# arangesh/TrackMPNN

Measured on AMD Instinct MI355X. Metric: graph_edges_per_sec_fwd_bwd, higher is better.
Workload: dtype f32; 1 GPU; C2 KITTI Car/RRC-shaped rolling windows: 7 frames, D_t~clip(Poisson(6),1,20), F=8 (2d), H=64, K=0, diff; 1 fwd per frame + 1 bwd per window; 16384 windows/GPU batched block-diagonally (64 distinct seeds tiled); windows_per_gpu=16384, rows_final=6762496, parallelism=sequence-dp1

## Files before the change

include/tmpnn.h:

```cpp
#ifndef TMPNN_H
#define TMPNN_H

#include <stddef.h>
#include <stdint.h>

#ifdef __cplusplus
extern "C" {
#endif

#define TMPNN_ABI_VERSION 4

#define TMPNN_OK 0
#define TMPNN_EINVAL (-1)
#define TMPNN_ELAUNCH (-2)
#define TMPNN_EWORKSPACE (-3)

typedef void* tmpnn_stream;
typedef void* tmpnn_event;

typedef struct tmpnn_seg_plan {
    int32_t T;
    int32_t I;
    int32_t nsplit;
    const int32_t* t_row;
// ... 82 lines not shown
int tmpnn_gru_fwd_head_parts(int H, int IN, int xmode);
int tmpnn_gru_fwd(const int32_t* rows, int R, int xmode, const int32_t* src, const int32_t* dst,
                  const float* msg, int ld_msg, int msg_compact, int IN, const float* h, int ld_h, int H,
                  const float* wih_t, const float* whh_t, const float* b_ih, const float* b_hh,
                  float* h_out, int ld_out, float* gates, size_t gate_plane,
                  const float* w_head, float* logit_part, size_t part_stride, tmpnn_stream stream);
int tmpnn_gru_bwd_data(const int32_t* rows, int R, int IN, const float* h, int ld_h, int H,
                       const float* w_ih, const float* w_hh,
                       const float* gates, size_t gate_plane, const float* d_hout, int ld_dhout,
                       const float* dy, const float* w_head,
                       float* d_msg, int ld_dmsg, float* d_h, int ld_dh,
                       const int32_t* add_src, const int32_t* add_dst, const float* add_msg, int ld_add,
                       tmpnn_stream stream);
size_t tmpnn_gru_bwd_weights_ws(int R, int IN, int H);
int tmpnn_gru_bwd_weights(const int32_t* rows, int R, int xmode, const int32_t* src, const int32_t* dst,
                          const float* msg, int ld_msg, int msg_compact, int IN,
                          const float* h, int ld_h, int H,
                          const float* gates, size_t gate_plane, const float* d_hout, int ld_dhout,
                          const float* dy, const float* w_head,
                          float* dW_ih, float* dW_hh, float* db_ih, float* db_hh,
                          void* ws, size_t ws_bytes, tmpnn_stream stream);

int tmpnn_gru_bwd_fused_available(int H, int IN, int xmode);
size_t tmpnn_gru_bwd_fused_ws(int R, int IN, int H);
int tmpnn_gru_bwd_fused(const int32_t* rows, int R, int xmode, const int32_t* src, const int32_t* dst,
                        const float* msg, int ld_msg, int msg_compact, int IN,
                        const float* h, int ld_h, int H, const float* w_ih, const float* w_hh,
                        const float* gates, size_t gate_plane, const float* d_hout, int ld_dhout,
                        const float* dy, const float* w_head,
                        float* d_msg, int ld_dmsg, float* d_h, int ld_dh,
                        const int32_t* add_src, const int32_t* add_dst, const float* add_msg, int ld_add,
                        float* dW_ih, float* dW_hh, float* db_ih, float* db_hh,
                        void* ws, size_t ws_bytes, tmpnn_stream stream);

int tmpnn_gru_fwd_tiles(const tmpnn_edge_tiles* tiles, int R, const float* proj, int ld_proj, const float* h, int ld_h, int H,
                        const float* whh_t, const float* b_ih, const float* b_hh, float* h_out, int ld_out, float* gates,
                        size_t gate_plane, const float* w_head, float* logit_part, size_t part_stride, tmpnn_stream stream);

int tmpnn_rows_linear(const int32_t* rows, int R, const float* in, int ld_in, int H, const float* wt, int NOUT,
                      float* out, int ld_out, tmpnn_stream stream);

int tmpnn_transpose(const float* in, int rows, int cols, float* out, tmpnn_stream stream);

int tmpnn_input_bn_fwd(const float* xdet, int ld_x, int F, int nd, const int32_t* seg_ptr,
                       const int32_t* seg_cnt, const int32_t* seg_of_det ,
                       int S, int H, int training,
                       const float* w1, const float* b1, const float* gamma, const float* beta,
                       float* running_mean, float* running_var,
                       const float* w2, const float* b2,
                       float* y_save, float* mean, float* rstd, float* ws_a ,
                       const int32_t* out_row, float* h_new, int ld_h, tmpnn_stream stream);
size_t tmpnn_input_bn_bwd_ws(int nd, int S, int H, int F);
int tmpnn_input_bn_bwd(const float* xdet, int ld_x, int F, int nd, const int32_t* seg_ptr,
                       const int32_t* seg_cnt, const int32_t* seg_of_det, int S, int H, int training,
                       const float* w1, const float* b1, const float* gamma, const float* beta,
                       const float* w2,
                       const float* y_save, const float* mean, const float* rstd,
                       const int32_t* out_row, const float* d_h, int ld_dh,
                       float* d_xdet, int ld_dx, float* d_xzero,
                       float* dw1, float* db1, float* dgamma, float* dbeta, float* dw2, float* db2,
                       float* ws, size_t ws_floats, tmpnn_stream stream);

int tmpnn_input_tf_supported(int H, int F, int max_seg_rows);
int tmpnn_input_tf_fwd(const float* xdet, const int64_t* x_rows, int ld_x, int F, int nd, const int32_t* seg_ptr, const int32_t* seg_cnt,
                       const int32_t* seg_of_det, int S, int max_seg_rows, int H, int training, const float* w1, const float* b1,
                       const float* gamma, const float* beta, float* running_mean, float* running_var, const float* w2,
// ... 219 lines not shown
```

trackmpnn_amd/_lib.py:

```python
from __future__ import annotations

import ctypes as C

import torch
import os
import re
from typing import Dict, List, Optional

_HERE = os.path.dirname(os.path.abspath(__file__))
LIB_PATH = os.environ.get('TMPNN_LIB_PATH') or os.path.join(_HERE, 'lib', 'libtmpnn.so')
HEADER_PATH = os.path.join(os.path.dirname(_HERE), 'include', 'tmpnn.h')

ABI_VERSION = 4

c_int = C.c_int
c_void_p = C.c_void_p
c_size_t = C.c_size_t
c_float = C.c_float


class CSegPlan(C.Structure):
    _fields_ = [('T', C.c_int32), ('I', C.c_int32), ('nsplit', C.c_int32), ('t_row', c_void_p), ('items', c_void_p),
                ('rowptr2', c_void_p), ('inc2', c_void_p), ('ws', c_void_p), ('ws_floats', c_size_t)]

# ... 60 lines not shown
    'tmpnn_segsum_bwd': (c_int, [_GP, c_void_p, c_int, c_void_p, c_int, c_int, c_int, c_void_p]),
    'tmpnn_att_fwd': (c_int, [_GP, c_void_p, c_void_p, c_int, c_int, c_int, c_void_p, c_void_p, c_void_p, c_float,
                              c_void_p, c_void_p, c_void_p, c_void_p, c_void_p, c_void_p, c_int, c_void_p]),
    'tmpnn_att_bwd_ws': (c_size_t, [c_int, c_int, c_int, c_int]),
    'tmpnn_att_index': (c_int, [_GP, c_void_p, c_void_p, c_void_p, c_void_p, c_void_p, c_void_p]),
    'tmpnn_att_bwd': (c_int, [_GP, c_void_p, c_void_p, c_void_p, c_int, c_int, c_int, c_void_p, c_void_p, c_void_p,
                              c_float, c_void_p, c_void_p, c_void_p, c_void_p, c_void_p, c_int, c_void_p, c_size_t,
                              c_void_p, c_int, c_void_p, c_void_p, c_void_p]),
    'tmpnn_att_bwd_heads': (c_int, [_GP, c_void_p, c_void_p, c_void_p, c_int, c_int, c_int, c_void_p, c_void_p,
                                    c_void_p, c_float, c_void_p, c_void_p, c_void_p, c_void_p, c_void_p, c_int, c_void_p,
                                    c_size_t, c_void_p, c_int, c_void_p, c_void_p, c_void_p]),
    'tmpnn_gru_fwd': (c_int, [c_void_p, c_int, c_int, c_void_p, c_void_p, c_void_p, c_int, c_int, c_int,
                              c_void_p, c_int, c_int, c_void_p, c_void_p, c_void_p, c_void_p,
                              c_void_p, c_int, c_void_p, c_size_t, c_void_p, c_void_p, c_size_t, c_void_p]),
    'tmpnn_gru_fwd_head_parts': (c_int, [c_int, c_int, c_int]),
    'tmpnn_gru_fwd_tiles': (c_int, [_TP, c_int, c_void_p, c_int, c_void_p, c_int, c_int, c_void_p, c_void_p, c_void_p,
                                    c_void_p, c_int, c_void_p, c_size_t, c_void_p, c_void_p, c_size_t, c_void_p]),
    'tmpnn_heads_finish': (c_int, [c_void_p, c_size_t, c_int, c_int, c_void_p, c_void_p, c_void_p, c_void_p, c_void_p, c_void_p]),
    'tmpnn_gru_bwd_data': (c_int, [c_void_p, c_int, c_int, c_void_p, c_int, c_int, c_void_p, c_void_p,
                                   c_void_p, c_size_t, c_void_p, c_int, c_void_p, c_void_p,
                                   c_void_p, c_int, c_void_p, c_int,
                                   c_void_p, c_void_p, c_void_p, c_int, c_void_p]),
    'tmpnn_gru_bwd_weights_ws': (c_size_t, [c_int, c_int, c_int]),
    'tmpnn_gru_bwd_weights': (c_int, [c_void_p, c_int, c_int, c_void_p, c_void_p, c_void_p, c_int, c_int, c_int,
                                      c_void_p, c_int, c_int, c_void_p, c_size_t, c_void_p, c_int, c_void_p, c_void_p,
                                      c_void_p, c_void_p, c_void_p, c_void_p, c_void_p, c_size_t, c_void_p]),
    'tmpnn_gru_bwd_fused_available': (c_int, [c_int, c_int, c_int]),
    'tmpnn_gru_bwd_fused_ws': (c_size_t, [c_int, c_int, c_int]),
    'tmpnn_gru_bwd_fused': (c_int, [c_void_p, c_int, c_int, c_void_p, c_void_p, c_void_p, c_int, c_int, c_int,
                                    c_void_p, c_int, c_int, c_void_p, c_void_p, c_void_p, c_size_t, c_void_p, c_int,
                                    c_void_p, c_void_p, c_void_p, c_int, c_void_p, c_int,
                                    c_void_p, c_void_p, c_void_p, c_int, c_void_p, c_void_p, c_void_p, c_void_p,
                                    c_void_p, c_size_t, c_void_p]),
    'tmpnn_rows_linear': (c_int, [c_void_p, c_int, c_void_p, c_int, c_int, c_void_p, c_int, c_void_p, c_int, c_void_p]),
    'tmpnn_transpose': (c_int, [c_void_p, c_int, c_int, c_void_p, c_void_p]),
    'tmpnn_input_bn_fwd': (c_int, [c_void_p, c_int, c_int, c_int, c_void_p, c_void_p, c_void_p, c_int, c_int, c_int,
                                   c_void_p, c_void_p, c_void_p, c_void_p, c_void_p, c_void_p, c_void_p, c_void_p,
                                   c_void_p, c_void_p, c_void_p, c_void_p, c_void_p, c_void_p, c_int, c_void_p]),
    'tmpnn_input_bn_bwd_ws': (c_size_t, [c_int, c_int, c_int, c_int]),
    'tmpnn_input_bn_bwd': (c_int, [c_void_p, c_int, c_int, c_int, c_void_p, c_void_p, c_void_p, c_int, c_int, c_int,
                                   c_void_p, c_void_p, c_void_p, c_void_p, c_void_p,
                                   c_void_p, c_void_p, c_void_p, c_void_p, c_void_p, c_int,
                                   c_void_p, c_int, c_void_p,
                                   c_void_p, c_void_p, c_void_p, c_void_p, c_void_p, c_void_p,
                                   c_void_p, c_size_t, c_void_p]),
    'tmpnn_input_tf_supported': (c_int, [c_int, c_int, c_int]),
    'tmpnn_input_tf_fwd': (c_int, [c_void_p, c_void_p, c_int, c_int, c_int, c_void_p, c_void_p, c_void_p, c_int, c_int, c_int, c_int,
                                   c_void_p, c_void_p, c_void_p, c_void_p, c_void_p, c_void_p, c_void_p, c_void_p,
                                   c_void_p, c_void_p, c_void_p, c_void_p, c_void_p, c_int, c_void_p]),
    'tmpnn_input_tf_bwd_ws': (c_size_t, [c_int, c_int, c_int, c_int, c_int]),
    'tmpnn_input_tf_bwd': (c_int, [c_void_p, c_void_p, c_int, c_int, c_int, c_void_p, c_void_p, c_void_p, c_int, c_int, c_int, c_int,
                                   c_void_p, c_void_p, c_void_p, c_void_p, c_void_p,
                                   c_void_p, c_void_p, c_void_p, c_void_p, c_void_p, c_int,
                                   c_void_p, c_int, c_void_p,
                                   c_void_p, c_void_p, c_void_p, c_void_p, c_void_p, c_void_p,
                                   c_void_p, c_size_t, c_void_p]),
    'tmpnn_heads_fwd': (c_int, [c_void_p, c_int, c_int, c_int, c_void_p, c_void_p, c_void_p, c_void_p, c_void_p,
                                c_void_p, c_void_p, c_void_p]),
    'tmpnn_heads_bwd_ws': (c_size_t, [c_int, c_int]),
    'tmpnn_heads_bwd': (c_int, [c_void_p, c_int, c_int, c_int, c_void_p, c_void_p, c_void_p, c_void_p, c_void_p,
                                c_void_p, c_void_p, c_void_p, c_int, c_int, c_void_p, c_void_p, c_void_p, c_void_p,
                                c_void_p, c_size_t, c_void_p]),
    'tmpnn_targets': (c_int, [_GP, c_void_p, c_void_p, c_void_p]),
    'tmpnn_ce_loss_ws': (c_size_t, [c_int]),
    'tmpnn_ce_loss_fwd': (c_int, [_GP, c_void_p, c_void_p, c_void_p, c_void_p, c_void_p, c_size_t, c_void_p]),
    'tmpnn_ce_loss_bwd': (c_int, [_GP, c_void_p, c_void_p, c_void_p, c_void_p, c_void_p, c_void_p, c_void_p]),
# ... 149 lines not shown
```

trackmpnn_amd/csrc/gru_bwd.hip:

```cpp
#include "gru_common.h"

namespace tmpnn {



template <int NT>
__global__ __launch_bounds__(256) void k_gru_bwd_data(GruBwdDataArgs a) {
    const int wave = threadIdx.x >> 6, lane = threadIdx.x & 63;
    const int c = lane & 31, half = lane >> 5;
    const int r0 = (blockIdx.x * 4 + wave) * 32;
    if (r0 >= a.R) return;
    const int H = a.H;
    const int vcol0 = blockIdx.y * (32 * NT);
    const bool is_dx = vcol0 < a.IN;
    const int n0 = is_dx ? vcol0 : vcol0 - a.IN;
    const float* __restrict__ W = is_dx ? a.w_ih : a.w_hh;
    const int ldw = is_dx ? a.IN : H;
    const int li = min(r0 + c, a.R - 1);
    const int row = a.rows[li];
    const size_t gp = a.gate_plane;

    f32x16 acc[NT];
#pragma unroll
    for (int t = 0; t < NT; ++t)
// ... 1741 lines not shown
    }
#undef TWO_STAGE
#undef TWO_GATHER_IDS
#undef TWO_ISSUE_GATHER
#undef TWO_ISSUE_MAIN
#undef TWO_SLICE
    float* sw = a.slab_w + (size_t)blockIdx.x * (3 * H) * (2 * H);
    if (HHS || role == 0) {
#pragma unroll
        for (int j = 0; j < 3; ++j)
#pragma unroll
            for (int reg = 0; reg < 16; ++reg) {
                const int jj = (jt0 + j) * 32 + acc_row(reg, half);
                sw[(size_t)jj * (2 * H) + role * H + tt * 32 + c32] = acc[j][reg];
            }
    }
    {
        float* red = lds;
#pragma unroll
        for (int j = 0; j < 3; ++j) {
            const float tot = bsum[j] + __shfl_xor(bsum[j], 32);
            if (half == 0) red[wave * 96 + j * 32 + c32] = tot;
        }
        __syncthreads();
        if (HHS && tt == 0 && half == 0) {
            float* sb = a.slab_b + (size_t)blockIdx.x * 6 * H;
#pragma unroll
            for (int j = 0; j < 3; ++j)
                sb[role * 3 * H + (jt0 + j) * 32 + c32] = red[wave * 96 + j * 32 + c32] + red[(wave + 1) * 96 + j * 32 + c32];
        }
    }
}


__global__ void k_gru_reduce_w(const float* __restrict__ slab_w, const float* __restrict__ slab_b, int n_rs,
                               int IN, int H, float* __restrict__ dW_ih, float* __restrict__ dW_hh,
                               float* __restrict__ db_ih, float* __restrict__ db_hh) {
    const int XH = IN + H;
    const size_t nW = (size_t)3 * H * XH;
    const size_t i = (size_t)blockIdx.x * blockDim.x + threadIdx.x;
    if (i < nW) {
        float s = 0.f;
        for (int k = 0; k < n_rs; ++k) s += slab_w[(size_t)k * nW + i];
        const int j = (int)(i / XH), col = (int)(i % XH);
        if (col < IN) dW_ih[(size_t)j * IN + col] += s;
        else dW_hh[(size_t)j * H + (col - IN)] += s;
    } else if (i < nW + (size_t)6 * H) {
        const int b = (int)(i - nW);
        float s = 0.f;
        for (int k = 0; k < n_rs; ++k) s += slab_b[(size_t)k * 6 * H + b];
        if (b < 3 * H) db_ih[b] += s;
        else db_hh[b - 3 * H] += s;
    }
}

__global__ void k_gru_reduce_w_half(const float* __restrict__ slab_w, const float* __restrict__ slab_b, int n_rs, int H,
                                    float* __restrict__ dW_ih, int ld_dwih, float* __restrict__ dW_hh,
                                    float* __restrict__ db_ih, float* __restrict__ db_hh, int full) {
    const int XH = 2 * H;
    const size_t nW = (size_t)3 * H * XH;
    const size_t i = (size_t)blockIdx.x * blockDim.x + threadIdx.x;
    if (i < nW) {
        const int j = (int)(i / XH), col = (int)(i % XH);
        if (col >= H && !full) return;
        float s = 0.f;
        for (int k = 0; k < n_rs; ++k) s += slab_w[(size_t)k * nW + i];
        if (col < H) dW_ih[(size_t)j * ld_dwih + col] += s;
        else dW_hh[(size_t)j * H + (col - H)] += s;
    } else if (full && i < nW + (size_t)6 * H) {
        const int b = (int)(i - nW);
        float s = 0.f;
        for (int k = 0; k < n_rs; ++k) s += slab_b[(size_t)k * 6 * H + b];
        if (b < 3 * H) db_ih[b] += s;
        else db_hh[b - 3 * H] += s;
    }
}

__global__ void k_fold_slabs_gru(const float* __restrict__ slabs, size_t stride, int nslab, float* __restrict__ out,
                                 size_t n) {
    const size_t i = (size_t)blockIdx.x * blockDim.x + threadIdx.x;
    if (i >= n) return;
    const int k0 = blockIdx.y * 32, k1 = min(nslab, k0 + 32);
    float s = 0.f;
#pragma unroll 8
    for (int k = k0; k < k1; ++k) s += slabs[(size_t)k * stride + i];
    out[(size_t)blockIdx.y * n + i] = s;
}


static int weights_variant_default() {
    static const int v = [] {
        if (!split_enabled()) return 0;
        const char* e = getenv("TMPNN_SPLIT_WEIGHTS");
        return (e && e[0] == '0') ? 0 : 1;
    }();
    return v;
}
static void plan_weights(int R, int IN, int H, int* n_rs, int* RS, int* NQ, int* NCH) {
    *NQ = 3 * H / 32;
    *NCH = (IN + H + 127) / 128;
    long per = (long)(*NQ) * (*NCH);
    long want = 4096 / per;
    if (want < 1) want = 1;
    long by_rows = (R + 63) / 64;
    long n = by_rows < want ? by_rows : want;
    if (n < 1) n = 1;
    long rs = (R + n - 1) / n;
    rs = (rs + 1) & ~1L;
    if (rs < 2) rs = 2;
    n = (R + rs - 1) / rs;
    if (n < 1) n = 1;
    *n_rs = (int)n;
    *RS = (int)rs;
}

}

using namespace tmpnn;

// ... 226 lines not shown
    } while (0)
#else
    TM_REQUIRE(!(xmode == 0 && fuse), "gru_bwd_fused: xmode 0 with a fused adjoint needs a TMPNN_KEEP_VARIANTS build");
#define LF(X, U, F)                                                                                          \
    do {                                                                                                     \
        if (!((X) == 0 && (F))) {                                                                            \
            TM_SHM_ONCE((k_gru_bwd_two<X, U, F>), shm);                                                      \
            hipLaunchKernelGGL((k_gru_bwd_two<X, U, F>), dim3(n_rs), dim3(512), shm, st, a, ntiles);         \
        }                                                                                                    \
    } while (0)
#endif
#define LU(X, F) do { if (up == 1) LF(X, 1, F); else if (up == 2) LF(X, 2, F); else LF(X, 3, F); } while (0)
    if (xmode == 0) { if (fuse) LU(0, true); else LU(0, false); }
    else            { if (fuse) LU(1, true); else LU(1, false); }
#undef LU
#undef LF
    int rc = check_launch("gru_bwd_fused");
    if (rc) return rc;
    const float* rw = slab_w;
    const float* rb = slab_b;
    int nred = n_rs;
    if (n_rs > 64) {
        const int ng = ceil_div(n_rs, 32);
        float* fw = fold;
        float* fb = fold + (size_t)ng * nW;
        hipLaunchKernelGGL(k_fold_slabs_gru, dim3(ceil_div((long)nW, 256), ng), dim3(256), 0, st, slab_w, nW, n_rs, fw, nW);
        hipLaunchKernelGGL(k_fold_slabs_gru, dim3(ceil_div((long)nB, 256), ng), dim3(256), 0, st, slab_b, nB, n_rs, fb, nB);
        if ((rc = check_launch("gru_fold"))) return rc;
        rw = fw; rb = fb; nred = ng;
    }
    hipLaunchKernelGGL(k_gru_reduce_w, dim3(ceil_div((long)(nW + nB), 256)), dim3(256), 0, st, rw, rb, nred, IN, H,
                       dW_ih, dW_hh, db_ih, db_hh);
    return check_launch("gru_reduce_w");
}

#ifdef TMPNN_KEEP_VARIANTS
int tmpnn_gru_bwd_weights_choice(void) { return weights_variant_default(); }
#endif

size_t tmpnn_gru_bwd_weights_ws(int R, int IN, int H) {
    if (R <= 0) return 0;
    int n_rs, RS, NQ, NCH;
    plan_weights(R, IN, H, &n_rs, &RS, &NQ, &NCH);
    if (weights_use_lds(IN, H)) n_rs = std::max(n_rs, weights_lds_blocks(R));
    if (weights_use_chunk(IN, H)) n_rs = std::max(n_rs, weights_chunk_slabs(R, IN, H));
    const size_t per = (size_t)3 * H * (IN + H) + (size_t)6 * H;
    return ((size_t)n_rs * per + reduce_slabs_ws_floats(n_rs, per)) * sizeof(float);
}

int tmpnn_gru_bwd_weights(const int32_t* rows, int R, int xmode, const int32_t* src, const int32_t* dst,
                          const float* msg, int ld_msg, int msg_compact, int IN, const float* h, int ld_h, int H,
                          const float* gates,
                          size_t gate_plane, const float* d_hout, int ld_dhout, const float* dy, const float* w_head,
                          float* dW_ih, float* dW_hh,
                          float* db_ih, float* db_hh, void* ws, size_t ws_bytes, tmpnn_stream stream) {
    return tmpnn_gru_bwd_weights_variant(rows, R, xmode, src, dst, msg, ld_msg, msg_compact, IN, h, ld_h, H, gates,
                                         gate_plane, d_hout, ld_dhout, dy, w_head, dW_ih, dW_hh, db_ih, db_hh, ws,
                                         ws_bytes, -1, stream);
}

int tmpnn_gru_bwd_weights_variant(const int32_t* rows, int R, int xmode, const int32_t* src, const int32_t* dst,
                                  const float* msg, int ld_msg, int msg_compact, int IN, const float* h, int ld_h, int H,
                                  const float* gates,
                                  size_t gate_plane, const float* d_hout, int ld_dhout, const float* dy,
                                  const float* w_head, float* dW_ih, float* dW_hh,
                                  float* db_ih, float* db_hh, void* ws, size_t ws_bytes, int variant,
// ... 100 lines not shown
```

trackmpnn_amd/functional.py:

```python
from __future__ import annotations

import contextlib
import ctypes
import os
from dataclasses import dataclass
from typing import Dict, List, Optional, Sequence, Tuple

import torch

from . import _lib
from .graph import CallPlan, dense_seg_plan, edge_tiles, win_plan

ATT_DROPOUT_P = 0.5
INPLACE_GRADS = os.environ.get('TMPNN_INPLACE_GRADS', '0') == '1'
FUSED_BWD = os.environ.get('TMPNN_FUSED_BWD', '1') == '1'
WIDE_OVERLAP = os.environ.get('TMPNN_WIDE_OVERLAP', '0') == '1' and os.environ.get('TMPNN_KEEP_VARIANTS', '0') == '1'
ATT_KMAX = 8
_SPLIT = os.environ.get('TMPNN_SPLIT', '1')[:1] != '0'

_VARIANTS = os.environ.get('TMPNN_KEEP_VARIANTS', '0') == '1'


def _variant(name: str, default: str) -> str:
    return os.environ.get(name, default) if _VARIANTS else default


WIDE_DW = _variant('TMPNN_WIDE_DW', '1') == '1'
WIDE_DET = _variant('TMPNN_WIDE_DET', '1') == '1'
WIDE = _variant('TMPNN_WIDE', '1') != '0' and _SPLIT
WIDE_TILED = _variant('TMPNN_WIDE_TILED', '1') != '0'
FWD_TILED = _variant('TMPNN_FWD_TILED', '1') != '0' and _SPLIT
FWD_TILE_ROWS = 16 if _variant('TMPNN_FWD_TILE_ROWS', '32') == '16' else 32
INPUT_TF = _variant('TMPNN_INPUT_TF', '1') != '0'
RECOMPUTE_GATES = _variant('TMPNN_RECOMPUTE_GATES', '0') == '1'
CONCAT_PROJ = _variant('TMPNN_CONCAT_PROJ', '1') != '0'
WIN_SEGSUM = _variant('TMPNN_SEGSUM_WIN', '0') == '1'
WIDE_FUSED_ADJOINT = _variant('TMPNN_WIDE_FUSED_ADJOINT', '1') != '0'
_aux_streams: Dict[torch.device, 'torch.cuda.Stream'] = {}


def _aux_stream(dev) -> Optional[int]:
    if not WIDE_OVERLAP or torch.cuda.is_current_stream_capturing():
        return None
    key = torch.device(dev)
    s = _aux_streams.get(key)
    if s is None:
        s = torch.cuda.Stream(key)
        _aux_streams[key] = s
# ... 444 lines not shown
    xmode = 2 if spec.msg_type == 'concat' else 1
    plane = N * H
    ws_e = lib.tmpnn_gru_bwd_weights_ws(E, IN_e, H)
    ws_n = lib.tmpnn_gru_bwd_weights_ws(Dn, H, H)
    use_fused_bwd = (FUSED_BWD and lib.tmpnn_gru_bwd_fused_available(H, H, 0)
                     and lib.tmpnn_gru_bwd_fused_available(H, IN_e, xmode))
    ws_f = max(lib.tmpnn_gru_bwd_fused_ws(E, IN_e, H), lib.tmpnn_gru_bwd_fused_ws(Dn, H, H)) if use_fused_bwd else 0
    ws_w = torch.empty((max(ws_e, ws_n, ws_f) // 4 + 1,), **opts)
    w_node, w_edge = P['output_transform_node.weight'], P['output_transform_edge.weight']
    for gi in range(G):
        f = f'factor_grus.{gi}.'
        hg = h_cat.data_ptr() + 4 * gi * H
        dog = (dh_up.data_ptr() + 4 * gi * H) if dh_up is not None else None
        dhg = d_hcat.data_ptr() + 4 * gi * H
        gp = gates[gi].data_ptr()
        es = es_all[gi]
        dyp = _lib.ptr(dy)
        wn = (w_node.data_ptr() + 4 * gi * H) if dy is not None else None
        we = (w_edge.data_ptr() + 4 * gi * H) if dy is not None else None
        fuse = K == 0
        if use_fused_bwd:
            _lib.call('tmpnn_gru_bwd_fused', g.det_row.data_ptr(), Dn, 0, None, None, es.data_ptr(), H, 1, H,
                      hg, GH, H, P[f + 'node_gru.weight_ih'].data_ptr(), P[f + 'node_gru.weight_hh'].data_ptr(),
                      gp, plane, dog, GH, dyp, wn, dmsg.data_ptr(), IN_e, dhg, GH, None, None, None, 0,
                      grads[f + 'node_gru.weight_ih'].data_ptr(), grads[f + 'node_gru.weight_hh'].data_ptr(),
                      grads[f + 'node_gru.bias_ih'].data_ptr(), grads[f + 'node_gru.bias_hh'].data_ptr(),
                      ws_w.data_ptr(), ws_w.numel() * 4, st)
            if saved.get('proj') and gi in saved['proj']:
                proj_s, whh_t_s = saved['proj'][gi]
                h_scr = _wide_workspace(4 * N * GH, dev, slot=2)
                _lib.call('tmpnn_gru_fwd_tiles', edge_tiles(g, FWD_TILE_ROWS).cref(), E, proj_s.data_ptr(), 3 * H, hg, GH, H,
                          whh_t_s.data_ptr(), P[f + 'edge_gru.bias_ih'].data_ptr(), P[f + 'edge_gru.bias_hh'].data_ptr(),
                          h_scr.data_ptr() + 4 * gi * H, GH, gp, plane, None, None, 0, st)
            _lib.call('tmpnn_gru_bwd_fused', g.edge_row.data_ptr(), E, xmode, g.src.data_ptr(), g.dst.data_ptr(),
                      None, 0, 0, IN_e, hg, GH, H,
                      P[f + 'edge_gru.weight_ih'].data_ptr(), P[f + 'edge_gru.weight_hh'].data_ptr(),
                      gp, plane, dog, GH, dyp, we, dmsg.data_ptr(), IN_e, dhg, GH,
                      g.src.data_ptr() if fuse else None, g.dst.data_ptr() if fuse else None,
                      dmsg.data_ptr() if fuse else None, IN_e,
                      grads[f + 'edge_gru.weight_ih'].data_ptr(), grads[f + 'edge_gru.weight_hh'].data_ptr(),
                      grads[f + 'edge_gru.bias_ih'].data_ptr(), grads[f + 'edge_gru.bias_hh'].data_ptr(),
                      ws_w.data_ptr(), ws_w.numel() * 4, st)
        else:
            _lib.call('tmpnn_gru_bwd_data', g.det_row.data_ptr(), Dn, H, hg, GH, H,
                      P[f + 'node_gru.weight_ih'].data_ptr(), P[f + 'node_gru.weight_hh'].data_ptr(),
                      gp, plane, dog, GH, dyp, wn, dmsg.data_ptr(), IN_e, dhg, GH, None, None, None, 0, st)
            _lib.call('tmpnn_gru_bwd_weights', g.det_row.data_ptr(), Dn, 0, None, None, es.data_ptr(), H, 1, H,
                      hg, GH, H, gp, plane, dog, GH, dyp, wn,
                      grads[f + 'node_gru.weight_ih'].data_ptr(), grads[f + 'node_gru.weight_hh'].data_ptr(),
                      grads[f + 'node_gru.bias_ih'].data_ptr(), grads[f + 'node_gru.bias_hh'].data_ptr(),
                      ws_w.data_ptr(), ws_w.numel() * 4, st)
            wide_det = bool(saved.get('wide')) and WIDE_DET
            if wide_det:
                wsb = int(lib.tmpnn_wide_gru_bwd_diff_ws(N, E, Dn, H))
                ws_wide = _wide_workspace(wsb, dev)
                aux = _aux_stream(dev)
                args = (saved['wide'][gi].data_ptr(), g.cref(), hg, GH, H, gp, plane, dog, GH, dyp, we, dhg, GH,
                        grads[f + 'edge_gru.weight_ih'].data_ptr(), grads[f + 'edge_gru.weight_hh'].data_ptr(),
                        grads[f + 'edge_gru.bias_ih'].data_ptr(), grads[f + 'edge_gru.bias_hh'].data_ptr(),
                        ws_wide.data_ptr(), wsb, st)
                evf = evj = None
                if aux is not None:
                    ef, ej = _aux_event_pair(dev)
                    evf, evj = ef.cuda_event, ej.cuda_event
                    if not evf or not evj:
                        aux = evf = evj = None
                _seg_plan_guard(g, dev, aux is not None)
                if fuse and WIDE_FUSED_ADJOINT:
                    _lib.call('tmpnn_wide_gru_bwd_diff_fused', *args[:-1], dmsg.data_ptr(), IN_e, st, aux, evf, evj)
                else:
                    if aux is not None:
                        _lib.call('tmpnn_wide_gru_bwd_diff_aux', *args, aux, evf, evj)
                    else:
                        _lib.call('tmpnn_wide_gru_bwd_diff', *args)
                    if fuse:
# ... 163 lines not shown
```

Measured before the change: 679.9 million graph-edges/s.

## Add zero-hidden-state edge GRU backward kernel for newly created edges

Newly created edges (those added for new detections) start with a zero hidden state, so their GRU backward needs no W_hh matmul, no dh propagation and no dW_hh accumulation. The edge backward is split so old edges go through the existing fused kernel and new edges use a specialised kernel that only computes d_msg, dW_ih and the biases, using b_hn in place of the W_hh·h term. This aims to cut MFMA work and memory traffic for that slice of edges, at the cost of an extra kernel launch and reduction per frame. It also relies on the assumption that new edges sit contiguously at the tail of the edge list.

```diff
diff --git a/include/tmpnn.h b/include/tmpnn.h
--- a/include/tmpnn.h
+++ b/include/tmpnn.h
@@ -138,6 +138,13 @@
                         const int32_t* add_src, const int32_t* add_dst, const float* add_msg, int ld_add,
                         float* dW_ih, float* dW_hh, float* db_ih, float* db_hh,
                         void* ws, size_t ws_bytes, tmpnn_stream stream);
+int tmpnn_gru_bwd_fused_zero_state_available(int H, int IN, int xmode);
+int tmpnn_gru_bwd_fused_zero_state(const int32_t* rows, int R, const int32_t* src, const int32_t* dst, int IN,
+                                   const float* h, int ld_h, int H, const float* w_ih, const float* b_hn,
+                                   const float* gates, size_t gate_plane, const float* d_hout, int ld_dhout,
+                                   const float* dy, const float* w_head, float* d_msg, int ld_dmsg,
+                                   float* dW_ih, float* db_ih, float* db_hh,
+                                   void* ws, size_t ws_bytes, tmpnn_stream stream);
 
 int tmpnn_gru_fwd_tiles(const tmpnn_edge_tiles* tiles, int R, const float* proj, int ld_proj, const float* h, int ld_h, int H,
                         const float* whh_t, const float* b_ih, const float* b_hh, float* h_out, int ld_out, float* gates,
diff --git a/trackmpnn_amd/_lib.py b/trackmpnn_amd/_lib.py
--- a/trackmpnn_amd/_lib.py
+++ b/trackmpnn_amd/_lib.py
@@ -116,6 +116,11 @@
                                     c_void_p, c_void_p, c_void_p, c_int, c_void_p, c_int,
                                     c_void_p, c_void_p, c_void_p, c_int, c_void_p, c_void_p, c_void_p, c_void_p,
                                     c_void_p, c_size_t, c_void_p]),
+    'tmpnn_gru_bwd_fused_zero_state_available': (c_int, [c_int, c_int, c_int]),
+    'tmpnn_gru_bwd_fused_zero_state': (c_int, [c_void_p, c_int, c_void_p, c_void_p, c_int, c_void_p, c_int, c_int,
+                                               c_void_p, c_void_p, c_void_p, c_size_t, c_void_p, c_int, c_void_p,
+                                               c_void_p, c_void_p, c_int, c_void_p, c_void_p, c_void_p, c_void_p,
+                                               c_size_t, c_void_p]),
     'tmpnn_rows_linear': (c_int, [c_void_p, c_int, c_void_p, c_int, c_int, c_void_p, c_int, c_void_p, c_int, c_void_p]),
     'tmpnn_transpose': (c_int, [c_void_p, c_int, c_int, c_void_p, c_void_p]),
     'tmpnn_input_bn_fwd': (c_int, [c_void_p, c_int, c_int, c_int, c_void_p, c_void_p, c_void_p, c_int, c_int, c_int,
diff --git a/trackmpnn_amd/csrc/gru_bwd.hip b/trackmpnn_amd/csrc/gru_bwd.hip
--- a/trackmpnn_amd/csrc/gru_bwd.hip
+++ b/trackmpnn_amd/csrc/gru_bwd.hip
@@ -1797,6 +1797,236 @@
     }
 }
 
+template <int UP>
+__global__ __launch_bounds__(512) void k_gru_bwd_zs(GruBwdFusedArgs a, const float* __restrict__ b_hn, int ntiles) {
+    constexpr int H = 64;
+    constexpr int SUB = 32 * 128;
+    constexpr int PA = 2 * SUB, PB = SUB;
+    constexpr int OFF_B = 3 * PA;
+    constexpr int BUF = OFF_B + 3 * PB;
+    extern __shared__ float lds[];
+    uint16_t* const lds16 = reinterpret_cast<uint16_t*>(lds);
+    const int tid = threadIdx.x;
+    const int wave = __builtin_amdgcn_readfirstlane(tid >> 6), lane = tid & 63;
+    const int role = wave >> 2, q = wave & 3;
+    const int j16 = lane & 15, kq = lane >> 4;
+    const int srow = 4 * wave + kq, f4 = 4 * j16;
+    const int n0 = 16 * q;
+    uint4 wq[6][3];
+#pragma unroll
+    for (int s6 = 0; s6 < 6; ++s6) {
+        const int ch = s6 < 4 ? 4 * kq + s6 : 16 + 4 * (s6 - 4) + kq;
+        float v[8];
+#pragma unroll
+        for (int i = 0; i < 8; ++i) v[i] = a.w_ih[(size_t)(8 * ch + i) * a.ld_wih + n0 + j16];
+        const Split8 sp = split8_arr(v);
+        wq[s6][0] = sp.p1; wq[s6][1] = sp.p2; wq[s6][2] = sp.p3;
+    }
+    const float headl = (UP & 2) ? a.up.w_head[lane] : 0.f;
+    const float4 bhn = *reinterpret_cast<const float4*>(b_hn + f4);
+    const int st0 = dui_off(srow, f4);
+    const int swzj = dui_swz(j16), rowj = (16 * role + j16) * 128;
+    const int half = lane >> 5, c32 = lane & 31;
+    const int jt0 = (q >> 1) * 3, tt = q & 1;
+    const int i16 = lane & 15, tq = i16 >> 2, tp = i16 & 3, tg = (lane >> 4) & 1;
+    const int trow = (8 * half + tq) * 128, tsw0 = (tq << 2) | (2 * half);
+    const int kofs = role * 2048;
+    int offA[3], offB;
+#pragma unroll
+    for (int j = 0; j < 3; ++j) {
+        const int col = (jt0 + j) * 32;
+        const int ch = ((col & 127) >> 3) + 2 * tg + (tp >> 1);
+        offA[j] = kofs + (col >> 7) * SUB + trow + ((ch ^ tsw0) << 3) + 4 * (tp & 1);
+    }
+    {
+        const int ch = ((tt * 32) >> 3) + 2 * tg + (tp >> 1);
+        offB = kofs + OFF_B + trow + ((ch ^ tsw0) << 3) + 4 * (tp & 1);
+    }
+    f32x16 acc[3];
+#pragma unroll
+    for (int j = 0; j < 3; ++j)
+#pragma unroll
+        for (int i = 0; i < 16; ++i) acc[j][i] = 0.f;
+    float bs_r[4] = {0.f, 0.f, 0.f, 0.f}, bs_z[4] = {0.f, 0.f, 0.f, 0.f};
+    float bs_n[4] = {0.f, 0.f, 0.f, 0.f}, bs_nr[4] = {0.f, 0.f, 0.f, 0.f};
+
+    const int G = gridDim.x;
+    const int nmine = (ntiles - (int)blockIdx.x + G - 1) / G;
+    struct { float4 dh, r, z, n, xa, xb; float dy; } raw;
+    float d0[4], tv[4];
+    auto row_of = [&](int tile, bool tvld, bool& vld) -> int {
+        const int lr = tile * 32 + srow;
+        vld = tvld && lr < a.R;
+        return vld ? lr : a.R - 1;
+    };
+#define ZS_SLICE(SL, img, vld)                                                                               \
+    do {                                                                                                     \
+        float o_[4];                                                                                         \
+        if ((SL) == 0) {                                                                                     \
+            const float dh_[4] = {raw.dh.x, raw.dh.y, raw.dh.z, raw.dh.w}, r_[4] = {raw.r.x, raw.r.y, raw.r.z, raw.r.w}; \
+            const float z_[4] = {raw.z.x, raw.z.y, raw.z.z, raw.z.w}, n_[4] = {raw.n.x, raw.n.y, raw.n.z, raw.n.w}; \
+            const float hn_[4] = {bhn.x, bhn.y, bhn.z, bhn.w};                                               \
+            _Pragma("unroll") for (int i = 0; i < 4; ++i) {                                                  \
+                float d_ = (UP & 1) ? dh_[i] : 0.f;                                                          \
+                if (UP & 2) d_ += raw.dy * __shfl(headl, f4 + i);                                            \
+                d0[i] = (vld) ? d_ : 0.f;                                                                    \
+                tv[i] = d0[i] * (1.0f - z_[i]) * (1.0f - n_[i] * n_[i]);                                     \
+                const float q_ = tv[i] * r_[i];                                                              \
+                o_[i] = q_ * hn_[i] * (1.0f - r_[i]);                                                        \
+                bs_r[i] += o_[i]; bs_n[i] += tv[i]; bs_nr[i] += q_;                                          \
+            }                                                                                                \
+            half_put((img), st0, PA, o_);                                                                    \
+        } else if ((SL) == 1) {                                                                              \
+            const float z_[4] = {raw.z.x, raw.z.y, raw.z.z, raw.z.w}, n_[4] = {raw.n.x, raw.n.y, raw.n.z, raw.n.w}; \
+            _Pragma("unroll") for (int i = 0; i < 4; ++i) {                                                  \
+                o_[i] = d0[i] * (0.0f - n_[i]) * z_[i] * (1.0f - z_[i]);                                     \
+                bs_z[i] += o_[i];                                                                            \
+            }                                                                                                \
+            half_put((img), st0 ^ 64, PA, o_);                                                               \
+        } else if ((SL) == 3) {                                                                              \
+            half_put((img), SUB + st0, PA, tv);                                                              \
+        } else if ((SL) == 5) {                                                                              \
+            const float xa_[4] = {raw.xa.x, raw.xa.y, raw.xa.z, raw.xa.w}, xb_[4] = {raw.xb.x, raw.xb.y, raw.xb.z, raw.xb.w}; \
+            _Pragma("unroll") for (int i = 0; i < 4; ++i) o_[i] = xa_[i] - xb_[i];                           \
+            half_put((img) + OFF_B, st0, PB, o_);                                                            \
+        }                                                                                                    \
+    } while (0)
+#define ZS_ISSUE_MAIN(SL, orow_)                                                                             \
+    do {                                                                                                     \
+        const size_t gp_ = a.gate_plane;                                                                     \
+        const float* g0_ = a.gates + (size_t)(orow_) * H + f4;                                               \
+        if ((SL) == 0) {                                                                                     \
+            if (UP & 1) raw.dh = *reinterpret_cast<const float4*>(a.up.d_hout + (size_t)(orow_) * a.up.ld_dhout + f4); \
+            if (UP & 2) raw.dy = a.up.dy[(orow_)];                                                           \
+            raw.r = TWO_LD4(g0_);                                                                            \
+        } else if ((SL) == 1) {                                                                              \
+            raw.n = TWO_LD4(g0_ + 2 * gp_);                                                                  \
+            raw.z = TWO_LD4(g0_ + gp_);                                                                      \
+        }                                                                                                    \
+    } while (0)
+#define ZS_ISSUE_GATHER(gs_, gd_)                                                                            \
+    do {                                                                                                     \
+        raw.xa = *reinterpret_cast<const float4*>(a.h + (size_t)(gs_) * a.ld_h + f4);                        \
+        raw.xb = *reinterpret_cast<const float4*>(a.h + (size_t)(gd_) * a.ld_h + f4);                        \
+    } while (0)
+
+    bool valid_cur, valid_n;
+    int gs_cur, gd_cur;
+    int orow_n;
+    {
+        bool v0, v1;
+        const int lp0 = row_of(blockIdx.x, true, v0);
+        const int o0 = a.rows[lp0];
+        gs_cur = a.src[lp0]; gd_cur = a.dst[lp0];
+        ZS_ISSUE_MAIN(0, o0); ZS_ISSUE_MAIN(1, o0); ZS_ISSUE_GATHER(gs_cur, gd_cur);
+        const int lp1 = row_of(blockIdx.x + G, 1 < nmine, v1);
+        const int o1 = a.rows[lp1];
+        ZS_SLICE(0, lds16, v0); ZS_ISSUE_MAIN(0, o1);
+        ZS_SLICE(1, lds16, v0); ZS_ISSUE_MAIN(1, o1);
+        ZS_SLICE(3, lds16, v0);
+        ZS_SLICE(5, lds16, v0);
+        valid_cur = v1;
+        gs_cur = a.src[lp1]; gd_cur = a.dst[lp1];
+        const int lp2 = row_of(blockIdx.x + 2 * G, 2 < nmine, valid_n);
+        orow_n = a.rows[lp2];
+    }
+    __syncthreads();
+
+    for (int it = 0; it < nmine; ++it) {
+        const int tile = blockIdx.x + it * G;
+        uint16_t* const cur = lds16 + (it & 1) * BUF;
+        uint16_t* const nxt = lds16 + ((it & 1) ^ 1) * BUF;
+        const int er = a.rows[min(tile * 32 + 16 * role + j16, a.R - 1)];
+        const bool el = tile * 32 + 16 * role + j16 < a.R;
+        f32x4 accd;
+#pragma unroll
+        for (int i = 0; i < 4; ++i) accd[i] = 0.f;
+#pragma unroll
+        for (int s6 = 0; s6 < 6; ++s6) {
+            uint4 bd[3];
+            const uint16_t* pd;
+            {
+                const int chunk = s6 < 4 ? 4 * kq + s6 : 4 * (s6 - 4) + kq;
+                pd = cur + (s6 >= 4 ? SUB : 0) + rowj + ((chunk ^ swzj) << 3);
+            }
+            if (s6 < 3) {
+                uint4 aw[3], bt[3];
+                {
+                    const uint16_t* p0 = cur + offB;
+                    const uint16_t* p1 = cur + (offB ^ 8) + 4 * 128;
+#pragma unroll
+                    for (int pc = 0; pc < 3; ++pc) {
+                        const uint2 u0 = lds_read_tr(p0 + pc * PB), u1 = lds_read_tr(p1 + pc * PB);
+                        bt[pc] = make_uint4(u0.x, u0.y, u1.x, u1.y);
+                    }
+                }
+                const uint16_t* p0 = cur + offA[s6];
+                const uint16_t* p1 = cur + (offA[s6] ^ 8) + 4 * 128;
+#pragma unroll
+                for (int pc = 0; pc < 3; ++pc) {
+                    const uint2 u0 = lds_read_tr(p0 + pc * PA), u1 = lds_read_tr(p1 + pc * PA);
+                    aw[pc] = make_uint4(u0.x, u0.y, u1.x, u1.y);
+                }
+                ZS_SLICE(s6, nxt, valid_cur);
+                ZS_ISSUE_MAIN(s6, orow_n);
+                acc[s6] = mfma32_c<0>(aw, bt, acc[s6]); acc[s6] = mfma32_c<1>(aw, bt, acc[s6]);
+                acc[s6] = mfma32_c<2>(aw, bt, acc[s6]); acc[s6] = mfma32_c<3>(aw, bt, acc[s6]);
+                acc[s6] = mfma32_c<4>(aw, bt, acc[s6]); acc[s6] = mfma32_c<5>(aw, bt, acc[s6]);
+            } else {
+                ZS_SLICE(s6, nxt, valid_cur);
+                if (s6 == 3) ZS_ISSUE_GATHER(gs_cur, gd_cur);
+            }
+#pragma unroll
+            for (int pc = 0; pc < 3; ++pc) bd[pc] = *reinterpret_cast<const uint4*>(pd + pc * PA);
+            accd = mfma16_c<0>(wq[s6], bd, accd); accd = mfma16_c<1>(wq[s6], bd, accd);
+            accd = mfma16_c<2>(wq[s6], bd, accd); accd = mfma16_c<3>(wq[s6], bd, accd);
+            accd = mfma16_c<4>(wq[s6], bd, accd); accd = mfma16_c<5>(wq[s6], bd, accd);
+            __builtin_amdgcn_sched_barrier(0);
+        }
+        {
+            bool vnn;
+            const int lp2 = row_of(tile + 2 * G, it + 2 < nmine, vnn);
+            gs_cur = a.src[lp2]; gd_cur = a.dst[lp2];
+            valid_cur = valid_n;
+            const int lp3 = row_of(tile + 3 * G, it + 3 < nmine, valid_n);
+            orow_n = a.rows[lp3];
+            (void)vnn;
+        }
+        int cofs = n0 + 4 * kq;
+        asm volatile("" : "+v"(cofs));
+        if (el) *reinterpret_cast<float4*>(a.d_msg + ((size_t)er * a.ld_dmsg + cofs)) =
+                    make_float4(accd[0], accd[1], accd[2], accd[3]);
+        __syncthreads();
+    }
+#undef ZS_ISSUE_GATHER
+#undef ZS_ISSUE_MAIN
+#undef ZS_SLICE
+    float* sw = a.slab_w + (size_t)blockIdx.x * (3 * H) * (2 * H);
+#pragma unroll
+    for (int j = 0; j < 3; ++j)
+#pragma unroll
+        for (int reg = 0; reg < 16; ++reg) {
+            const int jj = (jt0 + j) * 32 + acc_row(reg, half);
+            sw[(size_t)jj * (2 * H) + role * H + tt * 32 + c32] = acc[j][reg];
+        }
+    {
+        float* red = lds;
+        *reinterpret_cast<float4*>(red + srow * 256 + 0 * 64 + f4) = make_float4(bs_r[0], bs_r[1], bs_r[2], bs_r[3]);
+        *reinterpret_cast<float4*>(red + srow * 256 + 1 * 64 + f4) = make_float4(bs_z[0], bs_z[1], bs_z[2], bs_z[3]);
+        *reinterpret_cast<float4*>(red + srow * 256 + 2 * 64 + f4) = make_float4(bs_n[0], bs_n[1], bs_n[2], bs_n[3]);
+        *reinterpret_cast<float4*>(red + srow * 256 + 3 * 64 + f4) = make_float4(bs_nr[0], bs_nr[1], bs_nr[2], bs_nr[3]);
+        __syncthreads();
+        if (tid < 256) {
+            float s = 0.f;
+            for (int r = 0; r < 32; ++r) s += red[r * 256 + tid];
+            float* sb = a.slab_b + (size_t)blockIdx.x * 6 * H;
+            const int g = tid >> 6, c = tid & 63;
+            if (g < 3) sb[g * H + c] = s;
+            if (g != 2) sb[3 * H + (g == 3 ? 2 : g) * H + c] = s;
+        }
+    }
+}
+
 
 __global__ void k_gru_reduce_w(const float* __restrict__ slab_w, const float* __restrict__ slab_b, int n_rs,
                                int IN, int H, float* __restrict__ dW_ih, float* __restrict__ dW_hh,
@@ -1850,6 +2080,24 @@
 #pragma unroll 8
     for (int k = k0; k < k1; ++k) s += slabs[(size_t)k * stride + i];
     out[(size_t)blockIdx.y * n + i] = s;
+}
+
+__global__ void k_gru_reduce_w_zs(const float* __restrict__ slab_w, const float* __restrict__ slab_b, int n_rs, int H,
+                                  float* __restrict__ dW_ih, float* __restrict__ db_ih, float* __restrict__ db_hh) {
+    const size_t nI = (size_t)3 * H * H, nW = 2 * nI;
+    const size_t i = (size_t)blockIdx.x * blockDim.x + threadIdx.x;
+    if (i < nI) {
+        const size_t o = (i / H) * (2 * H) + (i % H);
+        float s = 0.f;
+        for (int k = 0; k < n_rs; ++k) s += slab_w[(size_t)k * nW + o] + slab_w[(size_t)k * nW + o + H];
+        dW_ih[i] += s;
+    } else if (i < nI + (size_t)6 * H) {
+        const int b = (int)(i - nI);
+        float s = 0.f;
+        for (int k = 0; k < n_rs; ++k) s += slab_b[(size_t)k * 6 * H + b];
+        if (b < 3 * H) db_ih[b] += s;
+        else db_hh[b - 3 * H] += s;
+    }
 }
 
 
@@ -2142,6 +2390,67 @@
     hipLaunchKernelGGL(k_gru_reduce_w, dim3(ceil_div((long)(nW + nB), 256)), dim3(256), 0, st, rw, rb, nred, IN, H,
                        dW_ih, dW_hh, db_ih, db_hh);
     return check_launch("gru_reduce_w");
+}
+
+int tmpnn_gru_bwd_fused_zero_state_available(int H, int IN, int xmode) {
+    return (H == 64 && IN == 64 && xmode == 1 && device_gives_160k()) ? 1 : 0;
+}
+
+int tmpnn_gru_bwd_fused_zero_state(const int32_t* rows, int R, const int32_t* src, const int32_t* dst, int IN,
+                                   const float* h, int ld_h, int H, const float* w_ih, const float* b_hn,
+                                   const float* gates, size_t gate_plane, const float* d_hout, int ld_dhout,
+                                   const float* dy, const float* w_head, float* d_msg, int ld_dmsg, float* dW_ih,
+                                   float* db_ih, float* db_hh, void* ws, size_t ws_bytes, tmpnn_stream stream) {
+    TM_REQUIRE(tmpnn_gru_bwd_fused_zero_state_available(H, IN, 1), "gru_bwd_fused_zero_state: H=%d IN=%d not supported", H, IN);
+    if (R == 0) return TMPNN_OK;
+    TM_REQUIRE(R > 0 && rows && src && dst && h && w_ih && b_hn && gates && d_msg && dW_ih && db_ih && db_hh,
+               "gru_bwd_fused_zero_state: null pointer");
+    TM_REQUIRE(d_hout != nullptr || dy != nullptr, "gru_bwd_fused_zero_state: no upstream gradient");
+    TM_REQUIRE(dy == nullptr || (w_head != nullptr && aligned16(w_head)),
+               "gru_bwd_fused_zero_state: dy needs a 16-byte aligned w_head");
+    TM_REQUIRE((ld_h & 3) == 0 && aligned16(h) && aligned16(gates) && (gate_plane & 3) == 0 && aligned16(w_ih) &&
+                   aligned16(b_hn) && (d_hout == nullptr || ((ld_dhout & 3) == 0 && aligned16(d_hout))) &&
+                   (ld_dmsg & 3) == 0 && aligned16(d_msg) && ld_dmsg >= IN && ld_h >= H,
+               "gru_bwd_fused_zero_state: rows must be 16-byte aligned");
+    const size_t need = tmpnn_gru_bwd_fused_ws(R, IN, H);
+    if (ws == nullptr || ws_bytes < need)
+        return set_error(TMPNN_EWORKSPACE, "gru_bwd_fused_zero_state: workspace %zu < %zu bytes", ws_bytes, need);
+    const int n_rs = fused_blocks(R);
+    const size_t nW = (size_t)3 * H * (IN + H), nB = (size_t)6 * H;
+    float* slab_w = reinterpret_cast<float*>(ws);
+    float* slab_b = slab_w + (size_t)n_rs * nW;
+    float* fold = slab_b + (size_t)n_rs * nB;
+    GruBwdFusedArgs a{rows, R, src, dst, nullptr, 0, 0, h, ld_h, w_ih, nullptr, gates, gate_plane,
+                      DhSrc{d_hout, ld_dhout, dy, w_head}, d_msg, ld_dmsg, nullptr, 0, nullptr, nullptr, nullptr, 0,
+                      slab_w, slab_b, IN};
+    const int ntiles = ceil_div(R, 32);
+    const size_t shm = 147456;
+    hipStream_t st = as_stream(stream);
+    const int up = (d_hout ? 1 : 0) | (dy ? 2 : 0);
+#define LZ(U)                                                                                                \
+    do {                                                                                                     \
+        TM_SHM_ONCE((k_gru_bwd_zs<U>), shm);                                                                 \
+        hipLaunchKernelGGL((k_gru_bwd_zs<U>), dim3(n_rs), dim3(512), shm, st, a, b_hn, ntiles);              \
+    } while (0)
+    if (up == 1) LZ(1); else if (up == 2) LZ(2); else LZ(3);
+#undef LZ
+    int rc = check_launch("gru_bwd_fused_zero_state");
+    if (rc) return rc;
+    const float* rw = slab_w;
+    const float* rb = slab_b;
+    int nred = n_rs;
+    if (n_rs > 64) {
+        const int ng = ceil_div(n_rs, 32);
+        float* fw = fold;
+        float* fb = fold + (size_t)ng * nW;
+        hipLaunchKernelGGL(k_fold_slabs_gru, dim3(ceil_div((long)nW, 256), ng), dim3(256), 0, st, slab_w, nW, n_rs, fw, nW);
+        hipLaunchKernelGGL(k_fold_slabs_gru, dim3(ceil_div((long)nB, 256), ng), dim3(256), 0, st, slab_b, nB, n_rs, fb, nB);
+        if ((rc = check_launch("gru_fold"))) return rc;
+        rw = fw; rb = fb; nred = ng;
+    }
+    hipLaunchKernelGGL(k_gru_reduce_w_zs, dim3(ceil_div((long)(3 * H * H + nB), 256)), dim3(256), 0, st, rw, rb, nred, H,
+                       dW_ih, db_ih, db_hh);
+    return check_launch("gru_reduce_w_zs");
 }
 
 #ifdef TMPNN_KEEP_VARIANTS
diff --git a/trackmpnn_amd/functional.py b/trackmpnn_amd/functional.py
--- a/trackmpnn_amd/functional.py
+++ b/trackmpnn_amd/functional.py
@@ -14,6 +14,7 @@
 ATT_DROPOUT_P = 0.5
 INPLACE_GRADS = os.environ.get('TMPNN_INPLACE_GRADS', '0') == '1'
 FUSED_BWD = os.environ.get('TMPNN_FUSED_BWD', '1') == '1'
+ZERO_STATE_BWD = os.environ.get('TMPNN_BWD_ZERO_STATE', '1') != '0'
 WIDE_OVERLAP = os.environ.get('TMPNN_WIDE_OVERLAP', '0') == '1' and os.environ.get('TMPNN_KEEP_VARIANTS', '0') == '1'
 ATT_KMAX = 8
 _SPLIT = os.environ.get('TMPNN_SPLIT', '1')[:1] != '0'
@@ -524,15 +525,29 @@
                 _lib.call('tmpnn_gru_fwd_tiles', edge_tiles(g, FWD_TILE_ROWS).cref(), E, proj_s.data_ptr(), 3 * H, hg, GH, H,
                           whh_t_s.data_ptr(), P[f + 'edge_gru.bias_ih'].data_ptr(), P[f + 'edge_gru.bias_hh'].data_ptr(),
                           h_scr.data_ptr() + 4 * gi * H, GH, gp, plane, None, None, 0, st)
-            _lib.call('tmpnn_gru_bwd_fused', g.edge_row.data_ptr(), E, xmode, g.src.data_ptr(), g.dst.data_ptr(),
-                      None, 0, 0, IN_e, hg, GH, H,
-                      P[f + 'edge_gru.weight_ih'].data_ptr(), P[f + 'edge_gru.weight_hh'].data_ptr(),
-                      gp, plane, dog, GH, dyp, we, dmsg.data_ptr(), IN_e, dhg, GH,
-                      g.src.data_ptr() if fuse else None, g.dst.data_ptr() if fuse else None,
-                      dmsg.data_ptr() if fuse else None, IN_e,
-                      grads[f + 'edge_gru.weight_ih'].data_ptr(), grads[f + 'edge_gru.weight_hh'].data_ptr(),
-                      grads[f + 'edge_gru.bias_ih'].data_ptr(), grads[f + 'edge_gru.bias_hh'].data_ptr(),
-                      ws_w.data_ptr(), ws_w.numel() * 4, st)
+            b_hn = P[f + 'edge_gru.bias_hh'].data_ptr() + 4 * 2 * H
+            E_old = E - (n - int(plan.new_det_row.numel())) if n > 0 else E
+            zs = (ZERO_STATE_BWD and n > 0 and K == 0 and xmode == 1 and 0 <= E_old < E and b_hn % 16 == 0
+                  and not (saved.get('proj') and gi in saved['proj'])
+                  and lib.tmpnn_gru_bwd_fused_zero_state_available(H, IN_e, xmode))
+            E_full = E_old if zs else E
+            if E_full > 0:
+                _lib.call('tmpnn_gru_bwd_fused', g.edge_row.data_ptr(), E_full, xmode, g.src.data_ptr(), g.dst.data_ptr(),
+                          None, 0, 0, IN_e, hg, GH, H,
+                          P[f + 'edge_gru.weight_ih'].data_ptr(), P[f + 'edge_gru.weight_hh'].data_ptr(),
+                          gp, plane, dog, GH, dyp, we, dmsg.data_ptr(), IN_e, dhg, GH,
+                          g.src.data_ptr() if fuse else None, g.dst.data_ptr() if fuse else None,
+                          dmsg.data_ptr() if fuse else None, IN_e,
+                          grads[f + 'edge_gru.weight_ih'].data_ptr(), grads[f + 'edge_gru.weight_hh'].data_ptr(),
+                          grads[f + 'edge_gru.bias_ih'].data_ptr(), grads[f + 'edge_gru.bias_hh'].data_ptr(),
+                          ws_w.data_ptr(), ws_w.numel() * 4, st)
+            if zs:
+                _lib.call('tmpnn_gru_bwd_fused_zero_state', g.edge_row.data_ptr() + 4 * E_old, E - E_old,
+                          g.src.data_ptr() + 4 * E_old, g.dst.data_ptr() + 4 * E_old, IN_e, hg, GH, H,
+                          P[f + 'edge_gru.weight_ih'].data_ptr(), b_hn, gp, plane, dog, GH, dyp, we,
+                          dmsg.data_ptr(), IN_e, grads[f + 'edge_gru.weight_ih'].data_ptr(),
+                          grads[f + 'edge_gru.bias_ih'].data_ptr(), grads[f + 'edge_gru.bias_hh'].data_ptr(),
+                          ws_w.data_ptr(), ws_w.numel() * 4, st)
         else:
             _lib.call('tmpnn_gru_bwd_data', g.det_row.data_ptr(), Dn, H, hg, GH, H,
                       P[f + 'node_gru.weight_ih'].data_ptr(), P[f + 'node_gru.weight_hh'].data_ptr(),
```

Measured after the change: 711.6 million graph-edges/s (median of 6 runs). +4.7%, better.
